# hackmad/pbrt-v3-rs

Measured on AMD Instinct MI355X. Metric: Mrays/s, higher is better.
Workload: dtype f32

## Files before the change

pbrt-v3-rs_amd/csrc/api.hip:

```cpp
#include "host_math.h"
#include "scene_host.h"
#include "traverse.h"
#include "texture.h"
#include <algorithm>
#include <cstdio>
#include <cstdlib>
#include <mutex>

static std::string g_last_error;
static std::mutex g_err_mu;

namespace phost {

int set_err(PbrtHipScene* s, int code, const std::string& msg) {
    if (s) s->err = msg;
    else { std::lock_guard<std::mutex> g(g_err_mu); g_last_error = msg; }
    return code;
}
int hip_fail(PbrtHipScene* s, hipError_t e, const char* what) {
    std::string m = std::string(what) + ": " + hipGetErrorString(e);
    (void)hipGetLastError();
    return set_err(s, e == hipErrorOutOfMemory ? PBRT_HIP_ERR_OOM : PBRT_HIP_ERR_DEVICE, m);
}
int ensure_buf(PbrtHipScene* s, DevBuf& b, size_t bytes) {
// ... 131 lines not shown
            const MaterialRec& m = s->materials[i];
            if (!m.none && (m.textured || m.bump_tex1)) key[i] = (uint16_t)std::min(jt++, kMaxTex - 1u);
            else { key[i] = (uint16_t)(T + std::min(jp++, kMaxPlain - 1u)); n_plain++; }
        }
        const uint32_t U = std::min(n_plain, kMaxPlain);
        if ((rc = upload_vec(s, key, &d.mat_key))) return rc;
        d.ms_tex_keys = T; d.ms_key_emit = T + U; d.ms_key_idle = T + U + 1u;
    }
    if (!s->textures.empty() || !s->mipmaps.empty()) {
        std::vector<TexRec> recs; std::vector<TexOp> ops;
        for (const PbrtHipScene::TextureHost& t : s->textures) {
            recs.push_back(TexRec{(uint32_t)ops.size(), (uint32_t)t.prog.size()});
            ops.insert(ops.end(), t.prog.begin(), t.prog.end());
        }
        std::vector<float> lut(PH_EWA_LUT_SIZE);
        for (int i = 0; i < PH_EWA_LUT_SIZE; i++) {
            const float r2 = (float)i / (float)(PH_EWA_LUT_SIZE - 1);
            lut[(size_t)i] = std::exp(-2.0f * r2) - std::exp(-2.0f);
        }
        if ((rc = upload_vec(s, recs, &d.textures))) return rc;
        if ((rc = upload_vec(s, ops, &d.tex_ops))) return rc;
        if ((rc = upload_vec(s, s->mipmaps, &d.mipmaps))) return rc;
        if ((rc = upload_vec(s, s->texels, &d.texels))) return rc;
        if ((rc = upload_vec(s, lut, &d.ewa_lut))) return rc;
    }
    if (s->emission_only.empty()) { if ((rc = upload_vec(s, s->lights, &d.lights))) return rc; }
    else {
        std::vector<LightRec> all(s->lights);
        all.insert(all.end(), s->emission_only.begin(), s->emission_only.end());
        if ((rc = upload_vec(s, all, &d.lights))) return rc;
    }
    if ((rc = upload_vec(s, s->light_dist, &d.light_dist))) return rc;
    d.n_lights = (uint32_t)s->lights.size();
    if ((rc = upload_vec(s, s->infinite_lights, &d.infinite_lights))) return rc;
    d.n_infinite = (uint32_t)s->infinite_lights.size();
    if ((rc = upload_vec(s, s->inst_recs, &d.instances))) return rc;
    d.n_instances = (uint32_t)s->inst_recs.size();
    if (!s->inst_recs.empty() && !s->top_items.empty() && d.tris) {
        const uint32_t n_top = (uint32_t)s->top_items.size();
        const uint32_t n_nodes = (uint32_t)(s->tree_dev_tris ? s->bvh.interior_nodes : s->bvh.nodes.size());
        void* extra = nullptr;
        PH_CHECK(s, hipMalloc(&extra, (size_t)n_top * 48)); s->owned.push_back(extra);
        hipLaunchKernelGGL(patch_inst_records_kernel, dim3((n_top + 255u) / 256u), dim3(256), 0, s->stream, const_cast<TriRec*>(d.tris), n_top, d.instances, static_cast<float*>(extra));
        if (n_nodes) hipLaunchKernelGGL(patch_leaf_refs_kernel, dim3((n_nodes + 255u) / 256u), dim3(256), 0, s->stream, const_cast<Node64*>(d.nodes), n_nodes, d.tris, n_top);
        PH_CHECK(s, hipGetLastError());
        d.inst_extra = static_cast<const float*>(extra);
    }
    hm::HaltonTables& ht = halton_tables();
    if ((rc = upload_vec(s, ht.perms, &d.halton_perms))) return rc;
    if ((rc = upload_vec(s, ht.primes, &d.primes))) return rc;
    if ((rc = upload_vec(s, ht.prime_sums, &d.prime_sums))) return rc;
    if ((rc = upload_vec(s, ht.magic, &d.prime_magic))) return rc;
    if ((rc = upload_vec(s, s->sobol32, &d.sobol32))) return rc;
    if ((rc = upload_vec(s, s->vdc, &d.vdc))) return rc;
    if ((rc = upload_vec(s, s->vdc_inv, &d.vdc_inv))) return rc;
    {
        void* dself = nullptr;
        PH_CHECK(s, hipMalloc(&dself, sizeof(DeviceScene)));
        s->owned.push_back(dself);
        d.self = reinterpret_cast<const DeviceScene*>(dself);
        PH_CHECK(s, hipMemcpyAsync(dself, &d, sizeof(DeviceScene), hipMemcpyHostToDevice, s->stream));
    }
    PH_CHECK(s, hipStreamSynchronize(s->stream));
    s->uploaded = true;
    return PBRT_HIP_OK;
}

int upload_light_distribution(PbrtHipScene* s, int light_strategy) {
    const size_t n = s->lights.size();
    int strat = (n == 1) ? 0 : light_strategy;
    if (s->light_strategy_uploaded == strat) return PBRT_HIP_OK;
    std::vector<float> f(n, 1.0f), cdf;
    float func_int = 0.0f;
    if (strat == 1) {
        const float wr = s->world_radius;
        for (size_t i = 0; i < n; i++) {
            const LightRec& l = s->lights[i];
            float p[3];
            for (int c = 0; c < 3; c++) {
                switch (l.type) {
                case PH_L_INFINITE: {
                    if (l.map_mip1) { float t[3]; hmip_lookup_triangle(s, s->mipmaps[l.map_mip1 - 1u], 0.5f, 0.5f, 0.5f, t); p[c] = hm::kPi * wr * wr * t[c]; break; }
                    float tx = l.L[c];
                    float v = tx * (1.0f - 0.0f) * (1.0f - 0.0f) + tx * (1.0f - 0.0f) * 0.0f + tx * 0.0f * (1.0f - 0.0f) + tx * 0.0f * 0.0f;
                    p[c] = hm::kPi * wr * wr * v;
                    break;
                }
                case PH_L_DISTANT: p[c] = l.L[c] * hm::kPi * wr * wr; break;
                case PH_L_POINT: p[c] = (hm::kPi * 4.0f) * l.L[c]; break;
                case PH_L_PROJECTION: case PH_L_GONIO: {
                    float t[3] = {1.0f, 1.0f, 1.0f};
                    if (l.map_mip1) hmip_lookup_triangle(s, s->mipmaps[l.map_mip1 - 1u], 0.5f, 0.5f, 0.5f, t);
                    p[c] = l.type == PH_L_PROJECTION ? t[c] * l.L[c] * (2.0f * hm::kPi) * (1.0f - l.cos_total_width) : (hm::kPi * 4.0f) * l.L[c] * t[c];
                    break;
                }
                case PH_L_SPOT: p[c] = l.L[c] * (2.0f * hm::kPi) * (1.0f - 0.5f * (l.cos_falloff_start + l.cos_total_width)); break;
                default: p[c] = (l.two_sided ? 2.0f : 1.0f) * l.L[c] * l.area * hm::kPi; break;
                }
            }
            f[i] = 0.212671f * p[0] + 0.715160f * p[1] + 0.072169f * p[2];
        }
    }
    if (n) hm::distribution1d(f, cdf, func_int);
    int rc;
    if ((rc = ensure_buf(s, s->d_ld_func, std::max<size_t>(n, 1) * 4))) return rc;
    if ((rc = ensure_buf(s, s->d_ld_cdf, (n + 1) * 4))) return rc;
    if (n) {
        PH_CHECK(s, hipMemcpy(s->d_ld_func.p, f.data(), n * 4, hipMemcpyHostToDevice));
        PH_CHECK(s, hipMemcpy(s->d_ld_cdf.p, cdf.data(), (n + 1) * 4, hipMemcpyHostToDevice));
    }
    s->ds.ld_func = (const float*)s->d_ld_func.p; s->ds.ld_cdf = (const float*)s->d_ld_cdf.p; s->ds.ld_func_int = func_int;
    s->light_strategy_uploaded = strat;
    return PBRT_HIP_OK;
}

int ensure_traversal_workspace(PbrtHipScene* s) {
    if (!s->trav_blocks) {
        hipDeviceProp_t prop;
        PH_CHECK(s, hipGetDeviceProperties(&prop, s->device));
        int per_cu = 0;
        PH_CHECK(s, hipOccupancyMaxActiveBlocksPerMultiprocessor(&per_cu, ph::traverse_kernel<false, false, 16, 32, 12, 6, false, true, 0, 6>, PH_TRAV_BLOCK, 0));
        per_cu = std::max(std::min(per_cu, 6), 1);
        s->trav_blocks = (uint32_t)(prop.multiProcessorCount * per_cu);
    }
    const uint32_t total_threads = s->trav_blocks * PH_TRAV_BLOCK;
    int rc;
    if ((rc = ensure_buf(s, s->d_counter, 64))) return rc;
    if ((rc = ensure_buf(s, s->d_error, 64))) return rc;
    if ((rc = ensure_buf(s, s->d_counts, 64 + 36 * 8))) return rc;
    const int stack_cap = s->inst_recs.empty() ? PH_MAX_STACK : 2 * PH_MAX_STACK;
    const int lds_depth = s->inst_recs.empty() ? 12 : 11;
    if ((rc = ensure_buf(s, s->d_spill, (size_t)(stack_cap - lds_depth) * total_threads * sizeof(uint2)))) return rc;
    return PBRT_HIP_OK;
}

template <bool COUNT, int LEAF_MIN, int REFILL_MIN, int LDS_DEPTH, int NODE_STEPS, bool INST, int ALPHA, int WPE, int ALPHA_MIN>
static void launch_traverse_shape(PbrtHipScene* s, int mode, uint32_t blocks, const ph::TravParams& p) {
    const dim3 g(blocks), b(PH_TRAV_BLOCK);
    if (mode == 2) hipLaunchKernelGGL((ph::traverse_kernel<false, COUNT, LEAF_MIN, REFILL_MIN, LDS_DEPTH, NODE_STEPS, INST, true, ALPHA, WPE, ALPHA_MIN>), g, b, 0, s->stream, s->ds, p);
    else if (mode == 1) hipLaunchKernelGGL((ph::traverse_kernel<true, COUNT, LEAF_MIN, REFILL_MIN, LDS_DEPTH, NODE_STEPS, INST, false, ALPHA, WPE, ALPHA_MIN>), g, b, 0, s->stream, s->ds, p);
    else hipLaunchKernelGGL((ph::traverse_kernel<false, COUNT, LEAF_MIN, REFILL_MIN, LDS_DEPTH, NODE_STEPS, INST, false, ALPHA, WPE, ALPHA_MIN>), g, b, 0, s->stream, s->ds, p);
}

void launch_traverse_kernel(PbrtHipScene* s, int mode, uint32_t blocks, const ph::TravParams& p_in) {
    ph::TravParams p = p_in;
    p.spill = (uint2*)s->d_spill.p; p.total_threads = s->trav_blocks * PH_TRAV_BLOCK; p.error_flag = (uint32_t*)s->d_error.p;
    p.counts = (unsigned long long*)s->d_counts.p;
#if PH_PHASE_CLOCK
    p.phase = (unsigned long long*)s->d_counts.p + 8;
#endif
    p.batch = PH_BATCH;
    const bool inst = !s->inst_recs.empty();
    const int alpha = !s->alpha_textures ? 0 : s->alpha_lean ? 1 : 2;
    if (s->count_traversal) {
        if (alpha == 0) { if (inst) launch_traverse_shape<true, PH_LEAF_MIN, PH_REFILL_MIN, PH_LDS_DEPTH, 1, true, 0, 0, 0>(s, mode, blocks, p); else launch_traverse_shape<true, PH_LEAF_MIN, PH_REFILL_MIN, PH_LDS_DEPTH, 1, false, 0, 0, 0>(s, mode, blocks, p); }
        else if (alpha == 1) { if (inst) launch_traverse_shape<true, PH_LEAF_MIN, PH_REFILL_MIN, PH_LDS_DEPTH, 1, true, 1, 0, 0>(s, mode, blocks, p); else launch_traverse_shape<true, PH_LEAF_MIN, PH_REFILL_MIN, PH_LDS_DEPTH, 1, false, 1, 0, 0>(s, mode, blocks, p); }
        else { if (inst) launch_traverse_shape<true, PH_LEAF_MIN, PH_REFILL_MIN, PH_LDS_DEPTH, 1, true, 2, 0, 0>(s, mode, blocks, p); else launch_traverse_shape<true, PH_LEAF_MIN, PH_REFILL_MIN, PH_LDS_DEPTH, 1, false, 2, 0, 0>(s, mode, blocks, p); }
        return;
    }
    if (alpha == 2) {
        if (inst) launch_traverse_shape<false, PH_LEAF_MIN, PH_REFILL_MIN, PH_LDS_DEPTH, 3, true, 2, 0, 12>(s, mode, blocks, p);
        else launch_traverse_shape<false, PH_LEAF_MIN, PH_REFILL_MIN, PH_LDS_DEPTH, 3, false, 2, 0, 12>(s, mode, blocks, p);
    } else if (alpha == 1) {
        if (inst) launch_traverse_shape<false, 16, 12, 11, 5, true, 1, 5, 12>(s, mode, blocks, p);
        else launch_traverse_shape<false, 24, 12, PH_LDS_DEPTH, 5, false, 1, 0, 12>(s, mode, blocks, p);
    } else if (inst) {
        launch_traverse_shape<false, 24, 12, 11, 5, true, 0, 5, 0>(s, mode, blocks, p);
    } else {
        launch_traverse_shape<false, 16, 32, 12, 6, false, 0, 6, 0>(s, mode, blocks, p);
    }
}

int launch_traverse(PbrtHipScene* s, bool anyhit, const void* d_rays, void* d_out, uint32_t n, float* kernel_ms) {
    if (kernel_ms) *kernel_ms = 0.0f;
    if (n == 0) return PBRT_HIP_OK;
    int rc;
    if ((rc = ensure_traversal_workspace(s))) return rc;
    const uint32_t blocks = std::min<uint32_t>(s->trav_blocks, (n + PH_TRAV_BLOCK - 1) / PH_TRAV_BLOCK);
    PH_CHECK(s, hipMemsetAsync(s->d_counter.p, 0, 4, s->stream));
    ph::TravParams p{};
    p.rays = (const ph::RayIn*)d_rays; p.out = d_out; p.n = n; p.n_ptr = nullptr; p.counter = (uint32_t*)s->d_counter.p;
    if (kernel_ms) PH_CHECK(s, hipEventRecord(s->ev0, s->stream));
    launch_traverse_kernel(s, anyhit ? 1 : 0, blocks, p);
    PH_CHECK(s, hipGetLastError());
    if (kernel_ms) {
        PH_CHECK(s, hipEventRecord(s->ev1, s->stream));
        PH_CHECK(s, hipEventSynchronize(s->ev1));
        PH_CHECK(s, hipEventElapsedTime(kernel_ms, s->ev0, s->ev1));
    }
    return PBRT_HIP_OK;
}

}

using namespace phost;

namespace hm {
M4 m4_inverse(const M4& a) {
    int indxc[4] = {0, 0, 0, 0}, indxr[4] = {0, 0, 0, 0}, ipiv[4] = {0, 0, 0, 0};
    float minv[4][4];
    std::memcpy(minv, a.m, sizeof(minv));
    for (int i = 0; i < 4; i++) {
        int irow = 0, icol = 0;
        float big = 0.0f;
        for (int j = 0; j < 4; j++)
            if (ipiv[j] != 1)
                for (int k = 0; k < 4; k++)
                    if (ipiv[k] == 0) { float av = fabs_p(minv[j][k]); if (av >= big) { big = av; irow = j; icol = k; } }
        ipiv[icol] += 1;
        if (irow != icol) for (int k = 0; k < 4; k++) std::swap(minv[irow][k], minv[icol][k]);
        indxr[i] = irow; indxc[i] = icol;
        float pivinv = 1.0f / minv[icol][icol];
        minv[icol][icol] = 1.0f;
        for (int j = 0; j < 4; j++) minv[icol][j] *= pivinv;
        for (int j = 0; j < 4; j++)
            if (j != icol) {
                float save = minv[j][icol];
                minv[j][icol] = 0.0f;
                for (int k = 0; k < 4; k++) minv[j][k] -= minv[icol][k] * save;
            }
    }
    for (int j = 3; j >= 0; j--)
        if (indxr[j] != indxc[j]) for (int k = 0; k < 4; k++) std::swap(minv[k][indxr[j]], minv[k][indxc[j]]);
    M4 r; std::memcpy(r.m, minv, sizeof(minv)); return r;
}
}

extern "C" {

int pbrt_hip_device_count(void) {
    return ph_guard(nullptr, "pbrt_hip_device_count", [&]() -> int {
    int n = 0;
    hipError_t e = hipGetDeviceCount(&n);
    if (e != hipSuccess) { (void)hipGetLastError(); return e == hipErrorNoDevice ? 0 : PBRT_HIP_ERR_DEVICE; }
    return n;
    });
}

PbrtHipScene* pbrt_hip_scene_create(int device_ordinal) {
    return ph_guard_ptr<PbrtHipScene>("pbrt_hip_scene_create", [&]() -> PbrtHipScene* {
    int n = pbrt_hip_device_count();
    if (n <= 0 || device_ordinal < 0 || device_ordinal >= n) {
        set_err(nullptr, PBRT_HIP_ERR_NO_DEVICE, "pbrt_hip_scene_create: no usable HIP device (this library has no CPU path)");
        return nullptr;
    }
    if (hipSetDevice(device_ordinal) != hipSuccess) { set_err(nullptr, PBRT_HIP_ERR_DEVICE, "hipSetDevice failed"); return nullptr; }
    PbrtHipScene* s = new PbrtHipScene();
    s->device = device_ordinal;
    if (hipStreamCreate(&s->stream) != hipSuccess || hipEventCreate(&s->ev0) != hipSuccess || hipEventCreate(&s->ev1) != hipSuccess) {
        set_err(nullptr, PBRT_HIP_ERR_DEVICE, "stream/event creation failed");
        delete s;
        return nullptr;
    }
    return s;
    });
}

void pbrt_hip_scene_destroy(PbrtHipScene* s) {
    ph_guard_void([&]() {
    if (!s) return;
    free_multi(s);
    (void)hipSetDevice(s->device);
    (void)hipStreamSynchronize(s->stream);
    free_wavefront(s);
    free_owned(s);
    free_tree_dev(s);
    for (DevBuf* b : {&s->d_ld_func, &s->d_ld_cdf, &s->d_counter, &s->d_spill, &s->d_error, &s->d_counts, &s->d_rays_tmp, &s->d_out_tmp})
        if (b->p) (void)hipFree(b->p);
    if (s->ev0) (void)hipEventDestroy(s->ev0);
    if (s->ev1) (void)hipEventDestroy(s->ev1);
    if (s->stream) (void)hipStreamDestroy(s->stream);
    delete s;
    });
}

const char* pbrt_hip_last_error(const PbrtHipScene* s) {
    if (s) return s->err.c_str();
    std::lock_guard<std::mutex> g(g_err_mu);
    return g_last_error.c_str();
}

namespace {
float roughness_to_alpha(float roughness) {
    roughness = roughness > 1e-3f ? roughness : 1e-3f;
    const float x = std::log(roughness);
    return 1.62142f + 0.819955f * x + 0.1734f * x * x + 0.0171201f * x * x * x + 0.000640711f * x * x * x * x;
}
bool clamp3(const float in[3], float out[3]) {
    for (int c = 0; c < 3; c++) out[c] = hm::clampf(in[c], 0.0f, hm::kInf);
    return !(out[0] == 0.0f && out[1] == 0.0f && out[2] == 0.0f);
}
LobeRec lobe(uint32_t kind, uint32_t type) { LobeRec l{}; l.kind = kind; l.type = type; l.eta_a = l.eta_b = 1.0f; return l; }
void set_tr(LobeRec& l, float ax, float ay) { l.ax = 0.001f > ax ? 0.001f : ax; l.ay = 0.001f > ay ? 0.001f : ay; }
enum : uint32_t { T_REFL = 1, T_TRANS = 2, T_DIFF = 4, T_GLOSSY = 8, T_SPEC = 16 };
int push_material(PbrtHipScene* s, MaterialRec& m, const std::vector<LobeRec>& lobes, bool general, uint32_t* out_id) {
    m.lobe_base = (uint32_t)s->lobes.size(); m.n_lobes = (uint32_t)lobes.size();
    s->lobes.insert(s->lobes.end(), lobes.begin(), lobes.end());
    s->materials.push_back(m);
    s->material_params.resize(s->materials.size());
    if (general) s->general_materials = true;
    if (out_id) *out_id = (uint32_t)s->materials.size() - 1;
    s->uploaded = false;
    return PBRT_HIP_OK;
}
}

// ... 959 lines not shown
```

pbrt-v3-rs_amd/csrc/traverse.h:

```cpp
#pragma once
#include "dmath.h"
#include "scene_types.h"

namespace ph {

struct alignas(16) RayIn { float ox, oy, oz, t_max, dx, dy, dz, time; };
struct alignas(16) HitOut { float t; uint32_t prim; float b0, b1, b2; uint32_t pad[3]; };

#ifndef PH_TRAV_BLOCK
#define PH_TRAV_BLOCK 256
#endif
#ifndef PH_LDS_DEPTH
#define PH_LDS_DEPTH 12
#endif
#define PH_MAX_STACK 64

#ifndef PH_STREAM_NT
#define PH_STREAM_NT 1
#endif
#if PH_STREAM_NT && defined(__HIP_DEVICE_COMPILE__)
typedef float ph_v4f __attribute__((ext_vector_type(4)));
static __device__ __forceinline__ float4 ph_stream_load(const float4* p) { const ph_v4f v = __builtin_nontemporal_load(reinterpret_cast<const ph_v4f*>(p)); return make_float4(v.x, v.y, v.z, v.w); }
static __device__ __forceinline__ uint32_t ph_stream_load(const uint32_t* p) { return __builtin_nontemporal_load(p); }
static __device__ __forceinline__ void ph_stream_store(float4 v, float4* p) { const ph_v4f w = {v.x, v.y, v.z, v.w}; __builtin_nontemporal_store(w, reinterpret_cast<ph_v4f*>(p)); }
// ... 400 lines not shown
            float t0, t1;
#if PH_NODE_PK
            ph_mask m0, m1;
            node_boxes(r, q0, q1, q2, m0, t0, m1, t1);
#if defined(__HIP_DEVICE_COMPILE__)
            const ph_mask m_neg = lanes(__builtin_amdgcn_ubfe(r.sgn, q3.z, 1u) != 0u);
#else
            const ph_mask m_neg = lanes(((r.sgn >> q3.z) & 1u) != 0u);
#endif
            const bool neg_axis = lane_of(m_neg);
            const uint32_t near_ref = neg_axis ? q3.y : q3.x, far_ref = neg_axis ? q3.x : q3.y;
            const bool near_hit = lane_of((m_neg & m1) | (~m_neg & m0)), far_hit = lane_of((m_neg & m0) | (~m_neg & m1));
            const float far_t = neg_axis ? t0 : t1;
#else
            bool h0, h1;
            h0 = box_test(r, r.nx() ? q0.y : q0.x, r.nx() ? q0.x : q0.y, r.ny() ? q0.w : q0.z, r.ny() ? q0.z : q0.w,
                               r.nz() ? q1.y : q1.x, r.nz() ? q1.x : q1.y, t0);
            h1 = box_test(r, r.nx() ? q1.w : q1.z, r.nx() ? q1.z : q1.w, r.ny() ? q2.y : q2.x, r.ny() ? q2.x : q2.y,
                               r.nz() ? q2.w : q2.z, r.nz() ? q2.z : q2.w, t1);
            h0 = h0 & (t0 < r.t_max);
            h1 = h1 & (t1 < r.t_max);
            const int neg_axis = (int)((r.sgn >> q3.z) & 1u);
            const uint32_t near_ref = neg_axis ? q3.y : q3.x, far_ref = neg_axis ? q3.x : q3.y;
            const bool near_hit = neg_axis ? h1 : h0, far_hit = neg_axis ? h0 : h1;
            const float far_t = neg_axis ? t0 : t1;
#endif
            if (COUNT && ah) {
                if (near_hit) { c_visits++; if (!far_hit) push(far_ref, __builtin_nanf("")); }
                else c_visits += 2;
            }
            if (near_hit) { cur = near_ref; if (far_hit) push(far_ref, far_t); }
            else if (far_hit) cur = far_ref;
            else cur = owe_pop();
            PHC_END(1);
        }
        }

        {
            const bool waiting = ALPHA && ALPHA_MIN > 0 && has_ray && alpha_wait;
            const bool at_leaf = has_ray && cur < PH_NEED_POP && (cur & PH_LEAF_BIT) && !waiting;
            const uint64_t lm = __ballot(at_leaf), am = (ALPHA && ALPHA_MIN > 0) ? __ballot(waiting) : 0ull;
            if ((lm | am) != 0ull) {
                const uint64_t nm = __ballot(has_ray && (cur == PH_NEED_POP || !(cur & PH_LEAF_BIT)));
                const bool fire_leaf = lm != 0ull && ((uint32_t)__popcll(lm) >= (uint32_t)LEAF_MIN || nm == 0ull || exhausted);
                const bool fire_alpha = am != 0ull && ((uint32_t)__popcll(am) >= (uint32_t)(ALPHA_MIN > 0 ? ALPHA_MIN : 1) || nm == 0ull || exhausted);
                if (fire_leaf || fire_alpha) {
#pragma unroll
                    for (int ls = 0; ls < PH_LEAF_STEPS; ls++)
                    if ((has_ray && cur < PH_NEED_POP && (cur & PH_LEAF_BIT) && !(ALPHA && ALPHA_MIN > 0 && alpha_wait) && (ls == 0 ? at_leaf : true) && fire_leaf) || (ls == 0 && waiting && fire_alpha)) {
                        PHC_BEGIN(9);
                        const uint32_t ti = INST ? (cur & ~(PH_LEAF_BIT | PH_LEAF_INST_HINT)) : (cur & ~PH_LEAF_BIT);
                        const float4* tp = reinterpret_cast<const float4*>(sc.tris + ti);
                        const float4 a = tp[0], b = tp[1], c = tp[2];
                        const bool hinted = INST && (cur & PH_LEAF_INST_HINT) != 0u;
                        float4 e0 = make_float4(0.0f, 0.0f, 0.0f, 0.0f), e1 = e0, e2 = e0;
                        if (INST && hinted) { const float4* ep = reinterpret_cast<const float4*>(sc.inst_extra) + 3u * (size_t)ti; e0 = ep[0]; e1 = ep[1]; e2 = ep[2]; }
                        const uint32_t flags = __float_as_uint(b.w);
                        bool last = (flags & PH_TRI_LAST) != 0;
                        const uint32_t next_ref = INST ? (((cur & ~PH_LEAF_INST_HINT) + 1u) | ((flags & PH_TRI_NEXT_INST) ? PH_LEAF_INST_HINT : 0u)) : cur + 1u;
                        float t, b0, b1, b2;
                        if (INST && (flags & PH_TRI_INSTANCE)) {
                            PHC_BEGIN(2);
                            if (!hinted) { const float4* ep = reinterpret_cast<const float4*>(sc.inst_extra) + 3u * (size_t)ti; e0 = ep[0]; e1 = ep[1]; e2 = ep[2]; }
                            const uint32_t iflags = __float_as_uint(c.y), iroot = __float_as_uint(c.x);
                            float w2i[16] = {e0.x, e0.y, e0.z, e0.w, e1.x, e1.y, e1.z, e1.w, e2.x, e2.y, e2.z, e2.w, 0.0f, 0.0f, 0.0f, 1.0f};
                            if (iflags & PH_INST_GENERAL) { const InstRec& I = sc.instances[__float_as_uint(a.w)]; for (int k = 12; k < 16; k++) w2i[k] = I.w2i[k]; }
                            world_tmax = r.t_max; cont_ref = last ? PH_INVALID_REF : next_ref;
                            in_inst = (__float_as_uint(a.w) + 1u) | ((r.sgn >> 3) << 30); inst_sp = sp; inst_hit = false;
                            inst_save[0][tid] = r.ox; inst_save[1][tid] = r.oy; inst_save[2][tid] = r.oz;
                            inst_save[3][tid] = r.ix; inst_save[4][tid] = r.iy; inst_save[5][tid] = r.iz; inst_save[6][tid] = r.sx; inst_save[7][tid] = r.sy; inst_save[8][tid] = r.sz;
                            const RayIn in = xf_ray(w2i, r, mk3(wdx, wdy, wdz), 0.0f);
                            ray_setup(r, in);
                            cur = PH_INVALID_REF;
                            if (iflags & PH_INST_SINGLE) cur = iroot;
                            else {
                                float tmin;
                                const bool h = box_test(r, r.nx() ? b.x : a.x, r.nx() ? a.x : b.x, r.ny() ? b.y : a.y, r.ny() ? a.y : b.y,
                                                        r.nz() ? b.z : a.z, r.nz() ? a.z : b.z, tmin);
                                if (h && tmin < r.t_max) cur = iroot;
                            }
                            PHC_END(2);
                        } else {
                        PHC_BEGIN(3);
                        if (COUNT) c_tris[(MIXED && ah) ? 1 : 0]++;
                        const bool second_meeting = ALPHA && ALPHA_MIN > 0 && alpha_wait;
                        alpha_wait = false;
                        if (tri_test(r, mk3(a.x, a.y, a.z), mk3(b.x, b.y, b.z), mk3(c.x, c.y, c.z), t, b0, b1, b2)) {
                            const uint32_t reject = ah ? (PH_TRI_BOGUS | PH_TRI_ALPHA0 | PH_TRI_SALPHA0) : (PH_TRI_BOGUS | PH_TRI_ALPHA0);
                            bool accept = !(flags & reject);
                            if (ALPHA && accept && (flags & PH_TRI_ALPHATEX)) {
                                if (ALPHA_MIN > 0 && !second_meeting) { alpha_wait = true; accept = false; }
                                else {
                                PHC_BEGIN(4);
                                accept = ALPHA == 1 ? alpha_accept_lean(sc, __float_as_uint(a.w), __float_as_uint(c.w), b0, b1, b2, ah) : alpha_accept(sc.self, ti, b0, b1, b2, ah ? 1u : 0u);
                                PHC_END(4);
                                }
                            }
                            if (accept) {
                                if (ah) occluded = true;
                                else {
                                    r.t_max = t; hit_tri = ti;
                                    if (!LEAN) { hit_prim = __float_as_uint(a.w); hb0 = b0; hb1 = b1; hb2 = b2; hit_cls = (flags >> PH_TRI_CLASS_SHIFT) & PH_TRI_KEY_MASK; }
                                    if (INST) { hit_inst = in_inst & 0x3FFFFFFFu; inst_hit = true; }
                                }
                            }
                        }
                        if (ALPHA && ALPHA_MIN > 0 && alpha_wait) { }
                        else if (ah && occluded) cur = PH_INVALID_REF;
                        else if (last) cur = owe_pop();
                        else cur = next_ref;
                        PHC_END(3);
                        }
                        PHC_END(9);
                    }
                }
            }
        }

        if (INST && has_ray && in_inst && cur == PH_INVALID_REF) {
            PHC_BEGIN(5);
            if (!(ah && occluded)) {
                const float t_new = inst_hit ? r.t_max : world_tmax;
                r.ox = inst_save[0][tid]; r.oy = inst_save[1][tid]; r.oz = inst_save[2][tid];
                r.ix = inst_save[3][tid]; r.iy = inst_save[4][tid]; r.iz = inst_save[5][tid]; r.sx = inst_save[6][tid]; r.sy = inst_save[7][tid]; r.sz = inst_save[8][tid];
                r.sgn = (r.ix < 0.0f ? 1u : 0u) | (r.iy < 0.0f ? 2u : 0u) | (r.iz < 0.0f ? 4u : 0u) | ((in_inst >> 30) << 3);
                r.t_max = t_new;
                in_inst = 0;
                cur = (cont_ref != PH_INVALID_REF) ? cont_ref : owe_pop();
            } else in_inst = 0;
            PHC_END(5);
        }

    }
    PHC_END(7);
#if PH_PHASE_CLOCK && defined(__HIP_DEVICE_COMPILE__)
    __syncthreads();
    if (tid < 36 && p.phase) atomicAdd(p.phase + tid, phc_lds[tid]);
#endif
    if (COUNT) {
        const int k0 = (!MIXED && ANYHIT) ? 3 : 0;
        atomicAdd(p.counts + k0 + 0, (unsigned long long)c_nodes[0]);
        atomicAdd(p.counts + k0 + 1, (unsigned long long)c_tris[0]);
        atomicAdd(p.counts + k0 + 2, (unsigned long long)c_rays[0]);
        if (MIXED) {
            atomicAdd(p.counts + 3, (unsigned long long)c_nodes[1]);
            atomicAdd(p.counts + 4, (unsigned long long)c_tris[1]);
            atomicAdd(p.counts + 5, (unsigned long long)c_rays[1]);
        }
        atomicAdd(p.counts + 6, (unsigned long long)c_visits);
        atomicAdd(p.counts + 7, (unsigned long long)c_culled);
    }
}

}
```

pbrt-v3-rs_amd/csrc/wavefront.hip:

```cpp
#define PH_OUTLINE_MATH 1
#include "host_math.h"
#include "pt_device.h"
#include "scene_host.h"
#include "spatial.h"
#include "bsdf_general.h"
#include "texture.h"
#include "raysort.h"
#include "phase_clock.h"
#include "matsort.h"
#include <algorithm>
#include <cstdlib>

namespace ph {

enum : uint32_t { F_EXT = 1u, F_PSH = 2u, F_PMIS = 4u, F_SPEC = 8u, F_NODIFF = 16u };

struct IterCounters {
    uint32_t n_cl, n_sh, n_live, head_cl, head_sh, pad[3];
};
struct DevStats { unsigned long long camera_rays, paths_total, paths_zero; };

struct TileInfo {
    int32_t tb[4];
    int32_t pb[4];
// ... 857 lines not shown
    const int kMaxNullSkips = 1024;
    const int n_iter_cap = s->has_none_material ? n_iter + kMaxNullSkips : n_iter;
    const bool mat_queues = s->general_materials || s->textured_materials;
    if ((rc = ensure_buf(s, w.d_ctr, (size_t)(n_iter_cap + 2) * sizeof(ph::IterCounters)))) return rc;
    if ((rc = ensure_buf(s, w.d_stats, 64 + 6 * PHC_N * 8))) return rc;
    if ((rc = ensure_buf(s, w.d_recL, (size_t)n_px * spp * 16))) return rc;
    if ((rc = ensure_buf(s, w.d_recpy, (size_t)n_px * spp * 4))) return rc;
    if ((rc = ensure_buf(s, w.d_rounded, (size_t)n_px))) return rc;
    PH_CHECK(s, hipMemsetAsync(w.d_rounded.p, 0, (size_t)n_px, s->stream));
    auto alloc_chunk = [&](size_t Bc) -> int {
        int r;
        if ((r = ensure_buf(s, w.d_rays_cl[0], 2 * Bc * sizeof(ph::RayIn)))) return r;
        if ((r = ensure_buf(s, w.d_rays_cl[1], 2 * Bc * sizeof(ph::RayIn)))) return r;
        if ((r = ensure_buf(s, w.d_hits, 2 * Bc * sizeof(ph::HitOut)))) return r;
        if ((r = ensure_buf(s, w.d_rays_sh, Bc * sizeof(ph::RayIn)))) return r;
        if ((r = ensure_buf(s, w.d_occ, Bc))) return r;
        if ((r = ensure_buf(s, w.d_live[0], Bc * 4))) return r;
        if ((r = ensure_buf(s, w.d_live[1], Bc * 4))) return r;
        for (DevBuf* b : {&w.d_sL, &w.d_sbeta, &w.d_sA, &w.d_sf2, &w.d_sbold, &w.d_sidx})
            if ((r = ensure_buf(s, *b, 2 * Bc * 16))) return r;
        if ((r = ensure_buf(s, w.d_sprev, 2 * Bc * 4))) return r;
        if ((r = ensure_buf(s, w.d_order, 3 * Bc * 4))) return r;
        if ((r = ensure_buf(s, w.d_keys_cl, 2 * Bc * 4))) return r;
        if ((r = ensure_buf(s, w.d_keys_sh, Bc * 4))) return r;
        if (s->textured_materials && (r = ensure_buf(s, w.d_tex_out, Bc * sizeof(TexOut)))) return r;
        if (mat_queues) {
            if ((r = ensure_buf(s, w.d_morder, Bc * 4))) return r;
            if ((r = ensure_buf(s, w.d_mkeys, Bc * 2))) return r;
        }
        return PBRT_HIP_OK;
    };
    int forced_oom = 0;
    if (const char* e = std::getenv("PBRT_HIP_TEST_CHUNK_OOM")) forced_oom = std::max(0, std::atoi(e));
    bool retried = false;
    for (;;) {
        if ((size_t)n_px * chunk_spp >= 0x7FFF0000ull) return set_err(s, PBRT_HIP_ERR_UNSUPPORTED, "render: tile range too large for one rank; use more tile_parts");
        if (forced_oom > 0) { forced_oom--; rc = set_err(s, PBRT_HIP_ERR_OOM, "render: out of device memory (forced by PBRT_HIP_TEST_CHUNK_OOM)"); }
        else rc = alloc_chunk((size_t)n_px * chunk_spp);
        if (rc == PBRT_HIP_OK) { if (retried) s->err.clear(); break; }
        retried = true;
        if (rc != PBRT_HIP_ERR_OOM || chunk_spp == 1) return rc;
        for (DevBuf* b : chunk_bufs()) if (b->p) { (void)hipFree(b->p); b->p = nullptr; b->bytes = 0; }
        chunk_spp = (chunk_spp + 1) / 2;
    }
    const size_t B = (size_t)n_px * chunk_spp;

    if ((rc = ensure_traversal_workspace(s))) return rc;
    const uint32_t n_heads = 8, head_chunk = 49152, sort_blocks = 1024;
    ph::RaySortParams sortp{};
    ph::RaySortGrid sort_grid{};
    if ((rc = ensure_buf(s, w.d_sort_bins, 2 * PH_SORT_KEYS * 4))) return rc;
    sortp.order = (uint32_t*)w.d_order.p; sortp.bin_start = (uint32_t*)w.d_sort_bins.p; sortp.bin_cursor = sortp.bin_start + PH_SORT_KEYS;
    sortp.keys_cl = (const uint32_t*)w.d_keys_cl.p; sortp.keys_sh = (const uint32_t*)w.d_keys_sh.p;
    for (int k = 0; k < 3; k++) {
        const float ext = s->bvh.root_hi[k] - s->bvh.root_lo[k];
        sort_grid.lo[k] = s->bvh.root_lo[k]; sort_grid.scale[k] = ext > 0.0f ? 1.0f / ext : 0.0f;
    }
    if ((rc = ensure_buf(s, w.d_heads, (size_t)(n_iter_cap + 2) * n_heads * 64))) return rc;
    ph::MatSortParams msp{};
    if (mat_queues) {
        if ((rc = ensure_buf(s, w.d_mbins, (size_t)(2 * PH_MS_BINS + 1) * 4))) return rc;
        msp.max_depth = max_depth; msp.mat_key = s->ds.mat_key; msp.key_emit = s->ds.ms_key_emit; msp.key_idle = s->ds.ms_key_idle;
        msp.tris = s->ds.tris; msp.meshes = s->ds.meshes; msp.hits = (const ph::HitOut*)w.d_hits.p;
        msp.keys = (uint16_t*)w.d_mkeys.p; msp.order = (uint32_t*)w.d_morder.p;
        msp.bin_start = (uint32_t*)w.d_mbins.p; msp.bin_cursor = msp.bin_start + PH_MS_BINS + 1;
    }

    ph::WfParams wp{};
    wp.cam = s->cam; wp.sp = s->sampler;
    wp.textured = s->textured_materials ? 1u : 0u; wp.cam_dev = nullptr;
    wp.any_rt = 0u;
    for (const MaterialRec& mr : s->materials) if (mr.rt_mode) wp.any_rt = 1u;
    if (s->textured_materials) {
        if ((rc = ensure_buf(s, w.d_cam, sizeof(CameraRec)))) return rc;
        PH_CHECK(s, hipMemcpyAsync(w.d_cam.p, &s->cam, sizeof(CameraRec), hipMemcpyHostToDevice, s->stream));
        wp.cam_dev = (const CameraRec*)w.d_cam.p;
    }
    for (int i = 0; i < 4; i++) wp.pixel_bounds[i] = pixel_bounds[i];
    wp.max_depth = max_depth; wp.rr_threshold = rr_threshold;
    wp.n_px = n_px; wp.px_xy = (const int2*)w.d_px.p;
    wp.rays_cl[0] = (ph::RayIn*)w.d_rays_cl[0].p; wp.rays_cl[1] = (ph::RayIn*)w.d_rays_cl[1].p;
    wp.hits_cl = (ph::HitOut*)w.d_hits.p; wp.rays_sh = (ph::RayIn*)w.d_rays_sh.p; wp.occ = (uint8_t*)w.d_occ.p;
    wp.live[0] = (uint32_t*)w.d_live[0].p; wp.live[1] = (uint32_t*)w.d_live[1].p;
    wp.ctr = (ph::IterCounters*)w.d_ctr.p; wp.stats = (ph::DevStats*)w.d_stats.p;
    for (int k = 0; k < 2; k++) {
        wp.s_L[k] = (float4*)w.d_sL.p + (size_t)k * B; wp.s_beta[k] = (float4*)w.d_sbeta.p + (size_t)k * B; wp.s_A[k] = (float4*)w.d_sA.p + (size_t)k * B;
        wp.s_f2[k] = (float4*)w.d_sf2.p + (size_t)k * B; wp.s_bold[k] = (float4*)w.d_sbold.p + (size_t)k * B; wp.s_idx[k] = (uint4*)w.d_sidx.p + (size_t)k * B;
        wp.s_prev[k] = (uint32_t*)w.d_sprev.p + (size_t)k * B;
    }
    wp.rec_L = (float4*)w.d_recL.p; wp.rec_py = (float*)w.d_recpy.p; wp.px_rounded = (uint8_t*)w.d_rounded.p;
    wp.sort_grid = sort_grid; wp.keys_cl = (uint32_t*)w.d_keys_cl.p; wp.keys_sh = (uint32_t*)w.d_keys_sh.p;
    wp.m_order = mat_queues ? (const uint32_t*)w.d_morder.p : nullptr; wp.m_bins = mat_queues ? (const uint32_t*)w.d_mbins.p : nullptr;

    if (spatial) { if ((rc = setup_spatial(s, wp.spatial))) return rc; }
    PH_CHECK(s, hipMemsetAsync(w.d_stats.p, 0, 64 + 6 * PHC_N * 8, s->stream));
    wp.phase = PH_PHASE_CLOCK ? (unsigned long long*)((char*)w.d_stats.p + 64) : nullptr;
    bool identity = true;
    for (const ph::TileInfo& t : w.tiles)
        if (t.tb[0] < pixel_bounds[0] || t.tb[1] < pixel_bounds[1] || t.tb[2] > pixel_bounds[2] || t.tb[3] > pixel_bounds[3]) { identity = false; break; }
    size_t ev = 0;
    hipEvent_t e_begin = get_event(s, ev++), e_end = get_event(s, ev++);
    if (!e_begin || !e_end) return set_err(s, PBRT_HIP_ERR_DEVICE, "hipEventCreate failed");
    struct Span { hipEvent_t a, b; int kind; };
    std::vector<Span> spans;
    auto timed = [&](int kind, auto&& launch) -> int {
        hipEvent_t a = get_event(s, ev++), b = get_event(s, ev++);
        if (!a || !b) return set_err(s, PBRT_HIP_ERR_DEVICE, "hipEventCreate failed");
        PH_CHECK(s, hipEventRecord(a, s->stream));
        launch();
        PH_CHECK(s, hipGetLastError());
        PH_CHECK(s, hipEventRecord(b, s->stream));
        spans.push_back({a, b, kind});
        return PBRT_HIP_OK;
    };
    PH_CHECK(s, hipEventRecord(e_begin, s->stream));
    uint64_t regular = 0, shadow = 0;
    std::vector<ph::IterCounters> hctr((size_t)n_iter_cap + 2);
    const uint32_t shade_blocks = (uint32_t)std::min<size_t>((B + 255) / 256, 256 * 16);
    wp.tex_out = nullptr;
    if (s->textured_materials) wp.tex_out = (TexOut*)w.d_tex_out.p;

    for (uint32_t s0 = 0; s0 < spp; s0 += chunk_spp) {
        const uint32_t cs = std::min(chunk_spp, spp - s0);
        wp.chunk_spp = cs; wp.s0 = s0; wp.B = n_px * cs; wp.identity_slots = identity ? 1u : 0u;
        PH_CHECK(s, hipMemsetAsync(w.d_ctr.p, 0, (size_t)(n_iter_cap + 2) * sizeof(ph::IterCounters), s->stream));
        PH_CHECK(s, hipMemsetAsync(w.d_heads.p, 0, (size_t)(n_iter_cap + 2) * n_heads * 64, s->stream));
        if (identity) hipLaunchKernelGGL(ph::preset_counters_kernel, dim3(1), dim3(1), 0, s->stream, wp.ctr, wp.stats, wp.B);
        if ((rc = timed(2, [&]() { hipLaunchKernelGGL(ph::raygen_kernel, dim3((wp.B + 255) / 256), dim3(256), 0, s->stream, s->ds, wp); }))) return rc;
        int iters_run = 0;
        for (int it = 0; it < n_iter_cap; it++) {
            ph::IterCounters* c = (ph::IterCounters*)w.d_ctr.p + it;
            if (it >= n_iter) {
                uint32_t live = 0;
                PH_CHECK(s, hipMemcpyAsync(&live, &c->n_live, 4, hipMemcpyDeviceToHost, s->stream));
                PH_CHECK(s, hipStreamSynchronize(s->stream));
                if (live == 0) break;
                if (it == n_iter_cap - 1) return set_err(s, PBRT_HIP_ERR_UNSUPPORTED, "render: a path crossed more than 1024 'none' surfaces");
            }
            iters_run = it + 1;
            ph::TravParams tp{};
            tp.rays = wp.rays_cl[it & 1]; tp.out = wp.hits_cl; tp.n = 0; tp.n_ptr = &c->n_cl; tp.counter = &c->head_cl;
            tp.heads = (uint32_t*)w.d_heads.p + (size_t)it * n_heads * 16; tp.n_heads = n_heads; tp.head_chunk = head_chunk;
            if (it > 0) {
                tp.rays2 = wp.rays_sh; tp.out2 = wp.occ; tp.n2_ptr = &c->n_sh;
                sortp.n_cl = &c->n_cl; sortp.n_sh = &c->n_sh;
                if ((rc = timed(3, [&]() {
                        (void)hipMemsetAsync(sortp.bin_start, 0, PH_SORT_KEYS * 4, s->stream);
                        hipLaunchKernelGGL(ph::raysort_hist_kernel, dim3(sort_blocks), dim3(PH_SORT_BLOCK), 0, s->stream, sortp);
                        hipLaunchKernelGGL(ph::raysort_scan_kernel, dim3(1), dim3(1024), 0, s->stream, sortp);
                        hipLaunchKernelGGL(ph::raysort_scatter_kernel, dim3(sort_blocks), dim3(PH_SORT_BLOCK), 0, s->stream, sortp);
                    }))) return rc;
                tp.order = sortp.order;
                if ((rc = timed(0, [&]() { launch_traverse_kernel(s, 2, s->trav_blocks, tp); }))) return rc;
            } else if ((rc = timed(0, [&]() { launch_traverse_kernel(s, 0, s->trav_blocks, tp); }))) return rc;
            if (mat_queues) {
                msp.s_idx = wp.s_idx[it & 1]; msp.n_live = &c->n_live;
                if ((rc = timed(2, [&]() {
                        (void)hipMemsetAsync(msp.bin_start, 0, (PH_MS_BINS + 1) * 4, s->stream);
                        hipLaunchKernelGGL(ph::matsort_hist_kernel, dim3(sort_blocks), dim3(PH_MS_BLOCK), 0, s->stream, msp);
                        hipLaunchKernelGGL(ph::matsort_scan_kernel, dim3(1), dim3(PH_MS_BINS), 0, s->stream, msp);
                        hipLaunchKernelGGL(ph::matsort_scatter_kernel, dim3(sort_blocks), dim3(PH_MS_BLOCK), 0, s->stream, msp);
                    }))) return rc;
            }
            if (s->textured_materials) {
                if ((rc = timed(2, [&]() {
                        const dim3 g(shade_blocks), b(PH_TEX_LDS_THREADS);
                        if (it == 0) {
                            if (s->simple_textures) hipLaunchKernelGGL((ph::texture_kernel<true, true, 3>), g, b, 0, s->stream, s->ds, wp, it);
                            else hipLaunchKernelGGL((ph::texture_kernel<false, true, 2>), g, b, 0, s->stream, s->ds, wp, it);
                        } else {
                            if (s->simple_textures) hipLaunchKernelGGL((ph::texture_kernel<true, false, 4>), g, b, 0, s->stream, s->ds, wp, it);
                            else hipLaunchKernelGGL((ph::texture_kernel<false, false, 3>), g, b, 0, s->stream, s->ds, wp, it);
                        }
                    }))) return rc;
            }
            if (spatial && (it < max_depth || s->has_none_material)) {
                if ((rc = timed(2, [&]() {
                        hipLaunchKernelGGL(ph::spatial_mark_kernel, dim3(shade_blocks), dim3(256), 0, s->stream, s->ds, wp, it);
                        hipLaunchKernelGGL(ph::spatial_compute_kernel, dim3(1024), dim3(PH_SPATIAL_BLOCK), 0, s->stream, s->ds, wp.spatial);
                    }))) return rc;
            }
            if ((rc = timed(2, [&]() {
                    if (s->textured_materials) {
                        if (s->general_materials) hipLaunchKernelGGL((ph::shade_kernel<true, true>), dim3(shade_blocks), dim3(256), 0, s->stream, s->ds, wp, it);
                        else hipLaunchKernelGGL((ph::shade_kernel<false, true>), dim3(shade_blocks), dim3(256), 0, s->stream, s->ds, wp, it);
                    } else if (s->general_materials) hipLaunchKernelGGL(ph::shade_kernel<true>, dim3(shade_blocks), dim3(256), 0, s->stream, s->ds, wp, it);
                    else hipLaunchKernelGGL(ph::shade_kernel<false>, dim3(shade_blocks), dim3(256), 0, s->stream, s->ds, wp, it);
                }))) return rc;
        }
        PH_CHECK(s, hipMemcpyAsync(hctr.data(), w.d_ctr.p, (size_t)(iters_run + 1) * sizeof(ph::IterCounters), hipMemcpyDeviceToHost, s->stream));
        PH_CHECK(s, hipStreamSynchronize(s->stream));
        for (int it = 0; it < iters_run; it++) { regular += hctr[it].n_cl; shadow += hctr[it].n_sh; }
    }

    ph::FilmParams fp{};
    fp.film = s->film; fp.tiles = (const ph::TileInfo*)w.d_tiles.p; fp.n_tiles = (uint32_t)w.tiles.size();
    fp.slot_w = w.slot_w; fp.slot_h = w.slot_h; fp.spp = spp; fp.n_px = n_px; fp.rec_L = wp.rec_L; fp.rec_py = wp.rec_py; fp.px_rounded = wp.px_rounded; fp.tile_buf = (float4*)d_tile_buffer;
    const uint64_t film_threads = (uint64_t)fp.n_tiles * w.slot_w * w.slot_h;
    if ((rc = timed(2, [&]() { hipLaunchKernelGGL(ph::film_tiles_kernel, dim3((uint32_t)((film_threads + 255) / 256)), dim3(256), 0, s->stream, fp); }))) return rc;
    PH_CHECK(s, hipEventRecord(e_end, s->stream));
    PH_CHECK(s, hipStreamSynchronize(s->stream));

    uint32_t flag = 0;
    PH_CHECK(s, hipMemcpy(&flag, s->d_error.p, 4, hipMemcpyDeviceToHost));
    if (flag) { (void)hipMemset(s->d_error.p, 0, 4); return set_err(s, PBRT_HIP_ERR_DEVICE, "traversal stack exceeded 64 entries (the reference panics here, bvh/mod.rs:185)"); }
    uint32_t sp_ctr[4] = {0, 0, 0, 0};
    if (spatial) {
        PH_CHECK(s, hipMemcpy(sp_ctr, w.d_sp_ctr.p, sizeof sp_ctr, hipMemcpyDeviceToHost));
        if (sp_ctr[ph::SP_OVERFLOW])
            return set_err(s, PBRT_HIP_ERR_OOM, "render: SpatialLightDistribution pool exhausted (" + std::to_string(sp_ctr[ph::SP_CLAIMED]) + " voxels x " +
                                                std::to_string(s->lights.size()) + " lights); use lightsamplestrategy power/uniform or a larger GPU memory budget");
    }
#if PH_PHASE_CLOCK
    {
        unsigned long long ph_[3 * PHC_N];
        PH_CHECK(s, hipMemcpy(ph_, (const char*)w.d_stats.p + 64, sizeof ph_, hipMemcpyDeviceToHost));
        static const char* names[11] = {"state+resolve", "surface+emission", "bsdf+textures", "sampler_dims", "light_pick", "light_sample_li", "f/pdf+shadow_ray", "mis_half", "bsdf_sample+rr", "queue_append", "whole_kernel"};
        for (int k = 0; k < 11; k++)
            std::fprintf(stderr, "SHADE_PHASE %-17s cycles %14llu (%5.1f %% of the kernel)  executions %12llu  mean active lanes %5.1f\n", names[k], ph_[k], ph_[10] ? 100.0 * (double)ph_[k] / (double)ph_[10] : 0.0,
                         ph_[PHC_N + k], ph_[PHC_N + k] ? (double)ph_[2 * PHC_N + k] / (double)ph_[PHC_N + k] : 0.0);
        unsigned long long pt_[3 * PHC_N];
        PH_CHECK(s, hipMemcpy(pt_, (const char*)w.d_stats.p + 64 + 3 * PHC_N * 8, sizeof pt_, hipMemcpyDeviceToHost));
        static const char* tnames[4] = {"hit+context", "bump", "lobe_colours", "whole_kernel"};
        for (int k = 0; k < 4; k++)
            std::fprintf(stderr, "TEXTURE_PHASE %-13s cycles %14llu (%5.1f %% of the kernel)  executions %12llu  mean active lanes %5.1f\n", tnames[k], pt_[k], pt_[3] ? 100.0 * (double)pt_[k] / (double)pt_[3] : 0.0,
                         pt_[PHC_N + k], pt_[PHC_N + k] ? (double)pt_[2 * PHC_N + k] / (double)pt_[PHC_N + k] : 0.0);
    }
#endif
    if (out_stats) {
        out_stats->light_distributions_created = sp_ctr[ph::SP_DONE];
        ph::DevStats ds;
        PH_CHECK(s, hipMemcpy(&ds, w.d_stats.p, sizeof(ds), hipMemcpyDeviceToHost));
        out_stats->camera_rays = ds.camera_rays; out_stats->regular_rays = regular; out_stats->shadow_rays = shadow;
        out_stats->paths_total = ds.paths_total; out_stats->paths_zero_radiance = ds.paths_zero;
        float ms = 0;
        PH_CHECK(s, hipEventElapsedTime(&ms, e_begin, e_end));
        out_stats->render_seconds = ms * 1e-3;
        double acc[4] = {0, 0, 0, 0};
        for (const Span& sp : spans) { float m = 0; if (hipEventElapsedTime(&m, sp.a, sp.b) == hipSuccess) acc[sp.kind] += m * 1e-3; }
        out_stats->extend_seconds = acc[0]; out_stats->shadow_seconds = acc[1]; out_stats->shade_seconds = acc[2] + acc[3];
        for (const Span& sp : spans) { if (sp.kind == 0) out_stats->extend_launches++; else if (sp.kind == 1) out_stats->shadow_launches++; }
    }
    return PBRT_HIP_OK;
}

int merge_tiles(PbrtHipScene* s, int tile_size, int parts, const void* const* d_bufs, float* out_xyz, float* out_weight) {
    if (!s->wf) s->wf = new Wavefront();
    Wavefront& w = *s->wf;
    const FilmRec& f = s->film;
    const TileGrid g = tile_grid(f, tile_size);
    const int cw = f.crop[2] - f.crop[0], ch = f.crop[3] - f.crop[1];
    const size_t npx = (size_t)std::max(cw, 0) * (size_t)std::max(ch, 0);
    if (npx == 0) return PBRT_HIP_OK;
    int rc;
    if ((rc = ensure_buf(s, w.d_xyz, npx * 12))) return rc;
    if ((rc = ensure_buf(s, w.d_w, npx * 4))) return rc;
    ph::MergeParams mp{};
    mp.film = f;
    for (int i = 0; i < 4; i++) mp.sb[i] = g.sb[i];
    mp.tile_size = tile_size; mp.ntx = g.ntx; mp.nty = g.nty; mp.parts = parts; mp.slot_w = g.slot_w; mp.slot_h = g.slot_h;
    for (int i = 0; i < parts; i++) mp.bufs[i] = (const float4*)d_bufs[i];
    mp.out_xyz = (float*)w.d_xyz.p; mp.out_w = (float*)w.d_w.p;
    hipLaunchKernelGGL(ph::merge_kernel, dim3((uint32_t)((npx + 255) / 256)), dim3(256), 0, s->stream, mp);
    PH_CHECK(s, hipGetLastError());
    PH_CHECK(s, hipMemcpyAsync(out_xyz, w.d_xyz.p, npx * 12, hipMemcpyDeviceToHost, s->stream));
    PH_CHECK(s, hipMemcpyAsync(out_weight, w.d_w.p, npx * 4, hipMemcpyDeviceToHost, s->stream));
    PH_CHECK(s, hipStreamSynchronize(s->stream));
    return PBRT_HIP_OK;
}

int spatial_voxels_touched(PbrtHipScene* s, std::vector<uint8_t>& touched, uint64_t* count) {
    if (!s->wf || !s->wf->d_vox_slot.p || !s->wf->n_vox) return PBRT_HIP_OK;
    PH_CHECK(s, hipSetDevice(s->device));
    std::vector<int32_t> slot(s->wf->n_vox);
    PH_CHECK(s, hipMemcpy(slot.data(), s->wf->d_vox_slot.p, slot.size() * 4, hipMemcpyDeviceToHost));
    if (touched.size() < slot.size()) touched.resize(slot.size(), 0);
    for (size_t v = 0; v < slot.size(); v++)
        if (slot[v] >= 0 && !touched[v]) { touched[v] = 1; (*count)++; }
    return PBRT_HIP_OK;
}

DevBuf& tile_buffer_of(PbrtHipScene* s) {
    if (!s->wf) s->wf = new Wavefront();
    return s->wf->d_tilebuf;
}

}

using namespace phost;

extern "C" {

int pbrt_hip_tile_buffer_floats(PbrtHipScene* s, int tile_size, int tile_part, int tile_parts, uint64_t* out_floats) {
    return ph_guard(s, "pbrt_hip_tile_buffer_floats", [&]() -> int {
    if (!s || !out_floats) return PBRT_HIP_ERR_INVALID_ARG;
    if (!s->have_film) return set_err(s, PBRT_HIP_ERR_STATE, "tile_buffer_floats: set_film first");
    if (tile_size <= 0 || tile_parts <= 0 || tile_part < 0 || tile_part >= tile_parts) return set_err(s, PBRT_HIP_ERR_INVALID_ARG, "tile_buffer_floats: bad partition");
    *out_floats = tile_buffer_floats_for(s, tile_size, tile_part, tile_parts);
    return PBRT_HIP_OK;
    });
}

int pbrt_hip_render_path_tiles_device(PbrtHipScene* s, int max_depth, float rr_threshold, int light_strategy, const int pixel_bounds[4], int tile_size,
                                      int tile_part, int tile_parts, void* d_tile_buffer, PbrtHipStats* out_stats) {
    return ph_guard(s, "pbrt_hip_render_path_tiles_device", [&]() -> int {
    int rc = check_render_args(s, max_depth, light_strategy, pixel_bounds, tile_size, tile_part, tile_parts);
    if (rc) return rc;
// ... 75 lines not shown
```

Before: 2326.

## Add wavefront-coherent packet traversal kernel for primary camera rays

Adds a packet traversal kernel in which each 64-lane wavefront walks the BVH together: rays are grouped by direction octant, node and triangle data are read through scalar (constant address space) loads, and the traversal stack holds one shared node plus a per-lane entry distance. The first bounce, which carries coherent camera rays, now uses this kernel whenever there are no instances, no alpha textures and counting is off. The aim is to replace per-lane divergent node fetches with uniform scalar loads and shared control flow. In exchange, lanes sit idle whenever their rays miss a node the packet still visits, and on stack overflow the group is halved and the rays re-run.

Measured after the change: 2355 (median of 6 runs). 1.3% higher.

```diff
diff --git a/pbrt-v3-rs_amd/csrc/api.hip b/pbrt-v3-rs_amd/csrc/api.hip
--- a/pbrt-v3-rs_amd/csrc/api.hip
+++ b/pbrt-v3-rs_amd/csrc/api.hip
@@ -307,6 +307,14 @@
     p.batch = PH_BATCH;
     const bool inst = !s->inst_recs.empty();
     const int alpha = !s->alpha_textures ? 0 : s->alpha_lean ? 1 : 2;
+    if (mode == 3) {
+        if (!s->count_traversal && !inst && alpha == 0) {
+            p.batch = 64;
+            hipLaunchKernelGGL((ph::traverse_packet_kernel<PH_LDS_DEPTH>), dim3(blocks), dim3(PH_TRAV_BLOCK), 0, s->stream, s->ds, p);
+            return;
+        }
+        mode = 0;
+    }
     if (s->count_traversal) {
         if (alpha == 0) { if (inst) launch_traverse_shape<true, PH_LEAF_MIN, PH_REFILL_MIN, PH_LDS_DEPTH, 1, true, 0, 0, 0>(s, mode, blocks, p); else launch_traverse_shape<true, PH_LEAF_MIN, PH_REFILL_MIN, PH_LDS_DEPTH, 1, false, 0, 0, 0>(s, mode, blocks, p); }
         else if (alpha == 1) { if (inst) launch_traverse_shape<true, PH_LEAF_MIN, PH_REFILL_MIN, PH_LDS_DEPTH, 1, true, 1, 0, 0>(s, mode, blocks, p); else launch_traverse_shape<true, PH_LEAF_MIN, PH_REFILL_MIN, PH_LDS_DEPTH, 1, false, 1, 0, 0>(s, mode, blocks, p); }
diff --git a/pbrt-v3-rs_amd/csrc/traverse.h b/pbrt-v3-rs_amd/csrc/traverse.h
--- a/pbrt-v3-rs_amd/csrc/traverse.h
+++ b/pbrt-v3-rs_amd/csrc/traverse.h
@@ -576,4 +576,157 @@
     }
 }
 
-}
+typedef uint32_t ph_u16 __attribute__((ext_vector_type(16)));
+typedef uint32_t ph_u8 __attribute__((ext_vector_type(8)));
+typedef uint32_t ph_u4 __attribute__((ext_vector_type(4)));
+template <typename V> PH_DEV V uniform_load(const void* base, size_t byte_off) {
+#if defined(__HIP_DEVICE_COMPILE__)
+    return *reinterpret_cast<__attribute__((address_space(4))) const V*>((__attribute__((address_space(4))) const char*)base + byte_off);
+#else
+    return *reinterpret_cast<const V*>(static_cast<const char*>(base) + byte_off);
+#endif
+}
+
+template <int LDS_DEPTH = PH_LDS_DEPTH>
+__global__ __launch_bounds__(PH_TRAV_BLOCK) void traverse_packet_kernel(DeviceScene sc, TravParams p) {
+    __shared__ uint2 lds_stack[LDS_DEPTH][PH_TRAV_BLOCK];
+    const uint32_t tid = threadIdx.x, lane = tid & 63u;
+    const uint32_t gtid = blockIdx.x * PH_TRAV_BLOCK + tid;
+    const uint64_t lane_lt = (lane == 0) ? 0ull : (~0ull >> (64 - lane));
+    const uint32_t n_rays = p.n_ptr ? *p.n_ptr : p.n;
+    uint32_t head_cur = p.n_heads > 1u ? blockIdx.x % p.n_heads : 0u, heads_dry = 0u;
+
+    for (;;) {
+        uint32_t base = 0, cnt = 0;
+        if (p.n_heads > 1u) {
+            while (cnt == 0u && heads_dry < p.n_heads) {
+                uint32_t b = 0;
+                if (lane == 0) b = atomicAdd(p.heads + 16u * head_cur, p.batch);
+                b = __shfl(b, 0);
+                const uint32_t chunk = b / p.head_chunk;
+                const uint64_t q = ((uint64_t)chunk * p.n_heads + head_cur) * p.head_chunk + (b - chunk * p.head_chunk);
+                if (q < (uint64_t)n_rays) { base = (uint32_t)q; cnt = ((uint32_t)q + p.batch < n_rays) ? p.batch : n_rays - (uint32_t)q; }
+                else { heads_dry++; head_cur = head_cur + 1u == p.n_heads ? 0u : head_cur + 1u; }
+            }
+        } else {
+            uint32_t b = 0;
+            if (lane == 0) b = atomicAdd(p.counter, p.batch);
+            b = __shfl(b, 0);
+            if (b < n_rays) { base = b; cnt = (b + p.batch < n_rays) ? p.batch : n_rays - b; }
+        }
+        if (cnt == 0u) break;
+
+        const bool has_ray = lane < cnt;
+        uint32_t ray_index = 0;
+        RayState r;
+        float t_max0 = 0.0f;
+        uint32_t hit_tri = 0xFFFFFFFFu;
+        if (has_ray) {
+            ray_index = p.order ? PH_STREAM_LOAD(p.order + base + lane) : base + lane;
+            const float4* rp = reinterpret_cast<const float4*>(p.rays + ray_index);
+            const float4 a = PH_STREAM_LOAD(rp), b = PH_STREAM_LOAD(rp + 1);
+            RayIn in; in.ox = a.x; in.oy = a.y; in.oz = a.z; in.t_max = a.w; in.dx = b.x; in.dy = b.y; in.dz = b.z; in.time = b.w;
+            ray_setup(r, in);
+            t_max0 = r.t_max;
+        } else { r = RayState{}; r.t_max = 0.0f; }
+
+        ph_mask todo = lanes(has_ray);
+        uint32_t max_lanes = 64u;
+        while (todo != 0ull && sc.root_ref != PH_INVALID_REF) {
+            const uint32_t first = (uint32_t)__builtin_ctzll(todo);
+            const uint32_t oct = __builtin_amdgcn_readfirstlane(__shfl(r.sgn & 7u, (int)first));
+            ph_mask grp = todo & lanes((r.sgn & 7u) == oct);
+            if ((uint32_t)__popcll(grp) > max_lanes) grp &= lanes((uint32_t)__popcll(grp & lane_lt) < max_lanes);
+            const bool nx = (oct & 1u) != 0u, ny = (oct & 2u) != 0u, nz = (oct & 4u) != 0u;
+            const bool mine = lane_of(grp);
+
+            ph_mask act;
+            {
+                float tmin = 0.0f;
+                const bool h = box_test(r, nx ? sc.root_hi[0] : sc.root_lo[0], nx ? sc.root_lo[0] : sc.root_hi[0], ny ? sc.root_hi[1] : sc.root_lo[1],
+                                        ny ? sc.root_lo[1] : sc.root_hi[1], nz ? sc.root_hi[2] : sc.root_lo[2], nz ? sc.root_lo[2] : sc.root_hi[2], tmin);
+                act = grp & lanes(h && tmin < r.t_max);
+            }
+            uint32_t cur = act != 0ull ? sc.root_ref : PH_INVALID_REF;
+            int sp = 0;
+            bool overflow = false;
+            while (cur != PH_INVALID_REF) {
+                if (!(cur & PH_LEAF_BIT)) {
+                    const ph_u16 q = uniform_load<ph_u16>(sc.nodes, (size_t)cur * sizeof(Node64));
+                    auto plane = [&](int k, bool neg) { const uint32_t lo = q[k], hi = q[k + 1]; return __uint_as_float(neg ? hi : lo); };
+                    float t0, t1;
+                    const bool h0 = box_test(r, plane(0, nx), plane(0, !nx), plane(2, ny), plane(2, !ny), plane(4, nz), plane(4, !nz), t0);
+                    const bool h1 = box_test(r, plane(6, nx), plane(6, !nx), plane(8, ny), plane(8, !ny), plane(10, nz), plane(10, !nz), t1);
+                    const ph_mask m0 = act & lanes(h0 && t0 < r.t_max), m1 = act & lanes(h1 && t1 < r.t_max);
+                    const bool neg_axis = ((oct >> q[14]) & 1u) != 0u;
+                    const uint32_t near_ref = neg_axis ? q[13] : q[12], far_ref = neg_axis ? q[12] : q[13];
+                    const ph_mask near_m = neg_axis ? m1 : m0, far_m = neg_axis ? m0 : m1;
+                    if (near_m != 0ull) {
+                        if (far_m != 0ull) {
+                            if (sp >= PH_MAX_STACK) {
+                                if (__popcll(grp) > 1) { overflow = true; break; }
+                                *p.error_flag = 1u;
+                            } else {
+                                const uint2 e = make_uint2(far_ref, lane_of(far_m) ? __float_as_uint(neg_axis ? t0 : t1) : 0x7fc00000u);
+                                if (sp < LDS_DEPTH) lds_stack[sp][tid] = e;
+                                else p.spill[(size_t)(sp - LDS_DEPTH) * p.total_threads + gtid] = e;
+                                sp++;
+                            }
+                        }
+                        cur = near_ref; act = near_m;
+                        continue;
+                    }
+                    if (far_m != 0ull) { cur = far_ref; act = far_m; continue; }
+                } else {
+                    uint32_t ti = cur & ~PH_LEAF_BIT;
+                    for (;;) {
+                        const ph_u8 qa = uniform_load<ph_u8>(sc.tris, (size_t)ti * sizeof(TriRec));
+                        const ph_u4 qb = uniform_load<ph_u4>(sc.tris, (size_t)ti * sizeof(TriRec) + 32u);
+                        const uint32_t flags = qa[7];
+                        if (lane_of(act)) {
+                            float t, b0, b1, b2;
+                            if (tri_test(r, mk3(__uint_as_float(qa[0]), __uint_as_float(qa[1]), __uint_as_float(qa[2])), mk3(__uint_as_float(qa[4]), __uint_as_float(qa[5]), __uint_as_float(qa[6])),
+                                         mk3(__uint_as_float(qb[0]), __uint_as_float(qb[1]), __uint_as_float(qb[2])), t, b0, b1, b2)
+                                && !(flags & (PH_TRI_BOGUS | PH_TRI_ALPHA0))) {
+                                r.t_max = t; hit_tri = ti;
+                            }
+                        }
+                        if (flags & PH_TRI_LAST) break;
+                        ti++;
+                    }
+                }
+                cur = PH_INVALID_REF;
+                while (sp > 0) {
+                    sp--;
+                    uint2 e;
+                    if (sp < LDS_DEPTH) { e = lds_stack[sp][tid]; asm volatile("; packet stack entry from LDS" : "+v"(e.x), "+v"(e.y)); }
+                    else { e = p.spill[(size_t)(sp - LDS_DEPTH) * p.total_threads + gtid]; asm volatile("; packet stack entry from the spill region" : "+v"(e.x), "+v"(e.y)); }
+                    act = lanes(__uint_as_float(e.y) < r.t_max);
+                    if (act != 0ull) { cur = __builtin_amdgcn_readfirstlane(e.x); break; }
+                }
+            }
+            if (overflow) {
+                if (mine) { r.t_max = t_max0; hit_tri = 0xFFFFFFFFu; }
+                max_lanes = (uint32_t)__popcll(grp) / 2u;
+                continue;
+            }
+            todo &= ~grp;
+        }
+
+        if (has_ray) {
+            uint32_t hit_prim = 0xFFFFFFFFu, hit_cls = 0u, tri_out = 0u;
+            float hb0 = 0.0f, hb1 = 0.0f, hb2 = 0.0f;
+            if (hit_tri != 0xFFFFFFFFu) {
+                const float4* tp = reinterpret_cast<const float4*>(sc.tris + hit_tri);
+                const float4 a = tp[0], b = tp[1], c = tp[2];
+                tri_bary(r, mk3(a.x, a.y, a.z), mk3(b.x, b.y, b.z), mk3(c.x, c.y, c.z), hb0, hb1, hb2);
+                hit_prim = __float_as_uint(a.w); hit_cls = (__float_as_uint(b.w) >> PH_TRI_CLASS_SHIFT) & PH_TRI_KEY_MASK; tri_out = hit_tri;
+            }
+            float4* hp = reinterpret_cast<float4*>(reinterpret_cast<HitOut*>(p.out) + ray_index);
+            PH_STREAM_STORE(make_float4(r.t_max, __uint_as_float(hit_prim), hb0, hb1), hp);
+            PH_STREAM_STORE(make_float4(hb2, __uint_as_float(tri_out), 0.0f, __uint_as_float(hit_cls)), hp + 1);
+        }
+    }
+}
+
+}
diff --git a/pbrt-v3-rs_amd/csrc/wavefront.hip b/pbrt-v3-rs_amd/csrc/wavefront.hip
--- a/pbrt-v3-rs_amd/csrc/wavefront.hip
+++ b/pbrt-v3-rs_amd/csrc/wavefront.hip
@@ -1033,7 +1033,7 @@
                     }))) return rc;
                 tp.order = sortp.order;
                 if ((rc = timed(0, [&]() { launch_traverse_kernel(s, 2, s->trav_blocks, tp); }))) return rc;
-            } else if ((rc = timed(0, [&]() { launch_traverse_kernel(s, 0, s->trav_blocks, tp); }))) return rc;
+            } else if ((rc = timed(0, [&]() { launch_traverse_kernel(s, 3, s->trav_blocks, tp); }))) return rc;
             if (mat_queues) {
                 msp.s_idx = wp.s_idx[it & 1]; msp.n_live = &c->n_live;
                 if ((rc = timed(2, [&]() {
```
